# tal-amir/fsw-gnn

Measured on AMD Instinct MI355X. Metric: edges*slices/sec FSW_conv forward, 1M-node/10M-edge, 256 slices, higher is better.
Workload: dtype f32; 1 GPU; BASELINE config 3: ER multigraph 1000000 nodes / 10000000 edges (9999936 after coalesce), 128 feat, 256 slices, FSW_conv(128->128, embed_dim=257), full forward incl. CSR build and Linear layer; nodes=1000000, edges=10000000, edges_coalesced=9999936, slices=256, features=128, parallelism=single GPU

## Files before the change

### fsw_gnn_amd/_lib.py

```python
import ctypes
import os

_HERE = os.path.dirname(os.path.abspath(__file__))
LIB_PATH = os.environ.get("FSW_HIP_LIBRARY") or os.path.join(_HERE, "libfsw_hip.so")

FSW_ABI_VERSION = 6
REG_MAX_DEG = 32
LDS_MAX_DEG = 2048
MID_SIZES = (40, 48, 64, 80, 96, 128, 160, 192, 256)
NUM_LDS_BINS = 3
NUM_HUB_BINS = 4
HUB_MAX_DEG = 32768
CART_SPLIT_LINES = 1
CART_SPLIT_BWD_LINES = 2
CART_SPLIT_W_LINES = 4
CART_W_MAX_LINE = 16384
BIN_MID0 = REG_MAX_DEG + 1
NUM_BINS = REG_MAX_DEG + 1 + len(MID_SIZES) + NUM_LDS_BINS + NUM_HUB_BINS + 1
NUM_STATS = 8
STAT_FLAGS, STAT_MAX_DEGREE, STAT_NUM_ZERO, STAT_NUM_REG, STAT_NUM_LDS, STAT_NUM_GLOBAL, STAT_NNZ, STAT_USER = 0, 1, 2, 3, 4, 5, 6, 7
BIN_BLOCK_ROWS, MAX_ROW_CHUNKS = 2048, 256
FLAG_INDEX_RANGE, FLAG_W_NONFINITE, FLAG_W_NEGATIVE, FLAG_X_NONFINITE = 1, 2, 4, 8

c_i64, c_i32, c_f32, c_vp, c_sz = ctypes.c_int64, ctypes.c_int32, ctypes.c_float, ctypes.c_void_p, ctypes.c_size_t
# ... 32 lines not shown
        ("unit_table", c_vp), ("ldt", c_i64), ("out", c_vp), ("ldo", c_i64), ("bias", c_vp), ("out_scale", ctypes.c_double),
        ("mass_fn", c_i32), ("flags", c_i32), ("mass_scale", ctypes.c_double), ("g", c_vp), ("ldg", c_i64),
        ("gkey", c_vp), ("ldk", c_i64), ("gfreq", c_vp), ("gw", c_vp), ("scratch", c_vp), ("scratch_bytes", c_sz),
    ]


_SIGNATURES = {
    "fsw_abi_version": (ctypes.c_int, []),
    "fsw_arch": (ctypes.c_char_p, []),
    "fsw_last_error": (ctypes.c_char_p, []),
    "fsw_graph_workspace_bytes": (c_sz, [c_i64, c_i64]),
    "fsw_graph_build_coalesced": (ctypes.c_int, [c_vp, c_vp, c_vp, c_vp, ctypes.c_int, c_i64, c_i64, c_i64, c_vp, c_vp, c_vp, c_vp, c_vp,
                                                 c_vp, c_vp, c_vp, c_vp, c_vp, c_sz, c_vp]),
    "fsw_graph_build": (ctypes.c_int, [c_vp, c_vp, c_vp, c_i64, c_i64, c_i64, c_i64, c_vp, c_vp, c_vp, c_vp, c_vp, c_vp, c_vp, c_vp, c_sz, c_vp]),
    "fsw_graph_build_two_level": (ctypes.c_int, [c_vp, c_vp, c_vp, c_i64, c_i64, c_i64, c_i64, c_vp, c_vp, c_vp, c_vp, c_vp, c_vp, c_vp, c_vp, c_sz, c_vp]),
    "fsw_project_f32": (ctypes.c_int, [c_vp, c_i64, ctypes.c_int, c_i64, c_vp, ctypes.c_int, c_i64, c_vp, c_i64, c_vp, c_i64, c_vp, c_vp]),
    "fsw_gemm_tn_workspace_bytes": (c_sz, [ctypes.c_int, ctypes.c_int]),
    "fsw_gemm_tn_f32": (ctypes.c_int, [c_vp, c_i64, c_vp, c_i64, c_i64, ctypes.c_int, ctypes.c_int, c_vp, c_i64, c_f32, c_vp, c_sz, c_vp]),
    "fsw_unit_table_rows": (c_sz, [ctypes.c_int]),
    "fsw_unit_coeff_table": (ctypes.c_int, [c_vp, ctypes.c_int, ctypes.c_int, c_vp, c_i64, c_vp]),
    "fsw_embed_scratch_bytes": (c_sz, [c_i64]),
    "fsw_embed_f32": (ctypes.c_int, [ctypes.POINTER(EmbedArgs), c_vp]),
    "fsw_conv_fused_lds_bytes": (c_sz, [ctypes.c_int, ctypes.c_int]),
    "fsw_packed_linear_floats": (c_sz, [ctypes.c_int, ctypes.c_int]),
    "fsw_pack_linear_f32": (ctypes.c_int, [c_vp, c_i64, ctypes.c_int, ctypes.c_int, ctypes.c_int, c_vp, c_vp, ctypes.c_int, c_vp, c_i64, c_vp]),
    "fsw_project_linear_f32": (ctypes.c_int, [c_vp, c_i64, ctypes.c_int, c_i64, c_vp, ctypes.c_int, c_i64, c_vp, c_i64,
                                              c_vp, ctypes.c_int, c_i64, c_vp, c_vp, c_i64, c_vp, c_vp, c_vp]),
    "fsw_conv_fused_f32": (ctypes.c_int, [ctypes.POINTER(EmbedArgs), c_vp, c_i64, c_vp, ctypes.c_int, c_vp, c_i64, ctypes.c_int,
                                          ctypes.c_int, c_f32, c_vp, c_i64, c_vp]),
    "fsw_add_bias_act_f32": (ctypes.c_int, [c_vp, c_i64, c_vp, c_i64, c_vp, c_i64, ctypes.c_int, ctypes.c_int, c_f32, c_vp]),
# ... 75 lines not shown
```

### fsw_gnn_amd/csrc/graph_build.hip

```cpp
#include <algorithm>
#include <atomic>
#include "fsw_common.h"
#include "graph_ws.h"

namespace fsw {

#ifndef FSW_RS_THREADS
#define FSW_RS_THREADS 512
#endif
constexpr int kRsThreads = FSW_RS_THREADS;
constexpr int kRsItems = kRsTile / kRsThreads;
static_assert(kRsThreads * kRsItems == kRsTile, "a tile is a whole number of rounds");
constexpr int kRsWaves = kRsThreads / kWave;

__device__ __forceinline__ int wave_inclusive_scan(int v) {
#pragma unroll
  for (int off = 1; off < kWave; off <<= 1) {
    int t = __shfl_up(v, off);
    if (lane_id() >= off) v += t;
  }
  return v;
}

__device__ __forceinline__ int block_exclusive_scan(int v, int* total) {
// ... 38 lines not shown
  }
}

__global__ void __launch_bounds__(kScanThreads) k_scan_apply(int32_t* __restrict__ data, int64_t n,
                                                             const int32_t* __restrict__ block_sums) {
  int64_t base = (int64_t)blockIdx.x * kScanTile + (int64_t)threadIdx.x * kScanItems;
  int v[kScanItems];
  int s = 0;
#pragma unroll
  for (int i = 0; i < kScanItems; ++i) {
    v[i] = base + i < n ? data[base + i] : 0;
    s += v[i];
  }
  int tot;
  int ex = block_exclusive_scan(s, &tot) + block_sums[blockIdx.x];
#pragma unroll
  for (int i = 0; i < kScanItems; ++i) {
    if (base + i < n) data[base + i] = ex;
    ex += v[i];
  }
}

static int exclusive_scan_i32(int32_t* data, int64_t n, int32_t* block_sums, int64_t block_sums_cap, hipStream_t stream) {
  const int64_t nb = ceil_div(n, kScanTile);
  FSW_REQUIRE(nb <= block_sums_cap, "exclusive_scan_i32: %lld elements need %lld block sums, the workspace holds %lld",
              (long long)n, (long long)nb, (long long)block_sums_cap);
  k_scan_partial<<<(unsigned)nb, kScanThreads, 0, stream>>>(data, n, block_sums);
  FSW_LAUNCH_CHECK();
  k_scan_block_sums<<<1, kScanThreads, 0, stream>>>(block_sums, nb);
  FSW_LAUNCH_CHECK();
// ... 184 lines not shown
      sval[lpos] = val[i];
    }
  }
  __syncthreads();
  const int64_t tile0 = (int64_t)blockIdx.x * kRsTile;
  const int count = (int)min((int64_t)kRsTile, num_edges - tile0);
  for (int i = threadIdx.x; i < count; i += kRsThreads) {
    const uint32_t k = skey[i];
    const uint32_t d = (k >> shift) & mask;
    const int64_t pos = (int64_t)gbase[d] + (i - dstart[d]);
    keys_out[pos] = k;
    vals_out[pos] = sval[i];
  }
}

template <class VAL>
__global__ void __launch_bounds__(256) k_finish_csr(const uint32_t* __restrict__ keys, const VAL* __restrict__ vals,
                                                    int64_t num_edges, int64_t num_rows, int32_t* __restrict__ rowptr,
                                                    int32_t* __restrict__ col, float* __restrict__ w) {
  for (int64_t i = (int64_t)blockIdx.x * blockDim.x + threadIdx.x; i <= num_edges; i += (int64_t)gridDim.x * blockDim.x) {
    const int64_t prev = i == 0 ? -1 : (int64_t)keys[i - 1];
    const int64_t cur = i == num_edges ? num_rows : (int64_t)keys[i];
    for (int64_t r = prev + 1; r <= cur && r <= num_rows; ++r) rowptr[r] = (int32_t)i;
    if (i < num_edges && cur < num_rows) {
      const VAL v = vals[i];
      col[i] = (int32_t)(uint32_t)v;
      if constexpr (sizeof(VAL) == 8) w[i] = __uint_as_float((uint32_t)(v >> 32));
    }
  }
}
// ... 71 lines not shown
      bin_cursor[c * FSW_NUM_BINS + b] = acc;
      if (b >= 1 && b <= FSW_REG_MAX_DEG) reg += cnt[b];
      if (b >= FSW_BIN_MID0 && b < FSW_BIN_HUB0) mid += cnt[b];
      acc += cnt[b];
    }
    bs[FSW_NUM_BINS] = acc;
    if (cnt[0]) atomicAdd(&stats[FSW_STAT_NUM_ZERO_DEG], cnt[0]);
    if (reg) atomicAdd(&stats[FSW_STAT_NUM_REG], reg);
    if (mid) atomicAdd(&stats[FSW_STAT_NUM_LDS], mid);
    int glob = 0;
    for (int b = FSW_BIN_HUB0; b <= FSW_BIN_GLOBAL; ++b) glob += cnt[b];
    if (glob) atomicAdd(&stats[FSW_STAT_NUM_GLOBAL], glob);
  }
}

__global__ void __launch_bounds__(256) k_bin_rows(const int32_t* __restrict__ rowptr, int64_t n, int64_t chunk_rows,
                                                  int32_t* __restrict__ bin_cursor, int32_t* __restrict__ perm,
                                                  int32_t* __restrict__ invperm) {
  __shared__ int lcount[FSW_NUM_BINS];
  __shared__ int lbase[FSW_NUM_BINS];
  if (threadIdx.x < FSW_NUM_BINS) lcount[threadIdx.x] = 0;
  __syncthreads();
  const int64_t r0 = (int64_t)blockIdx.x * kBinRowsPerBlock + threadIdx.x;
  int bin[kBinItems], rank[kBinItems];
#pragma unroll
  for (int i = 0; i < kBinItems; ++i) {
    const int64_t r = r0 + (int64_t)i * 256;
    const bool valid = r < n;
    bin[i] = valid ? degree_bin(rowptr[r + 1] - rowptr[r]) : 0;
    const unsigned long long peers = match_bin(bin[i], valid);
// ... 4 lines not shown
  }
  __syncthreads();
  const int64_t chunk = ((int64_t)blockIdx.x * kBinRowsPerBlock) / chunk_rows;
  if (threadIdx.x < FSW_NUM_BINS && lcount[threadIdx.x])
    lbase[threadIdx.x] = atomicAdd(&bin_cursor[chunk * FSW_NUM_BINS + threadIdx.x], lcount[threadIdx.x]);
  __syncthreads();
#pragma unroll
  for (int i = 0; i < kBinItems; ++i) {
    const int64_t r = r0 + (int64_t)i * 256;
    if (r < n) {
      const int pos = lbase[bin[i]] + rank[i];
      perm[pos] = (int32_t)r;
      if (invperm) invperm[r] = pos;
    }
  }
}

static int key_bits(int64_t range_a) {
  int keybits = 1;
  while ((1ll << keybits) <= range_a) ++keybits;
  return keybits;
}

template <class VAL, bool EID>
static int radix_sort_pairs(const int64_t* first_a, const int64_t* first_b, const float* edge_w, bool from_keys,
                            int64_t num_edges, int64_t range_a, int64_t range_b, int32_t* stats, GraphWs& g, int* cur_io,
                            hipStream_t stream, int lo_bit = 0, int max_bits = 8, int* last_bits = nullptr) {
  const int keybits = key_bits(range_a) - lo_bit;
  const int npass = (keybits + max_bits - 1) / max_bits;
  const int bits = (keybits + npass - 1) / npass;
  if (last_bits) *last_bits = bits;
  const int64_t ntiles = ceil_div(num_edges, kRsTile);
  int cur = *cur_io;
  for (int pass = 0; pass < npass; ++pass) {
    const int shift = lo_bit + pass * bits;
    const int ndigits = 1 << bits;
// ... 79 lines not shown
    col[p] = (int32_t)senders[eid[i]];
    w[p] = (float)wsum;
  }
}

__global__ void __launch_bounds__(256) k_rowptr_from_keys(const uint32_t* __restrict__ keyc, const int32_t* __restrict__ nnz_ptr,
                                                          int64_t num_rows, int32_t* __restrict__ rowptr) {
  const int64_t nnz = *nnz_ptr;
  for (int64_t i = (int64_t)blockIdx.x * blockDim.x + threadIdx.x; i <= nnz; i += (int64_t)gridDim.x * blockDim.x) {
    const int64_t prev = i == 0 ? -1 : (int64_t)keyc[i - 1];
    const int64_t cur = i == nnz ? num_rows : (int64_t)keyc[i];
    for (int64_t r = prev + 1; r <= cur && r <= num_rows; ++r) rowptr[r] = (int32_t)i;
  }
}

static int finish_bins(int32_t* rowptr, int64_t num_rows, int64_t chunk_rows, int32_t* perm, int32_t* invperm, int32_t* bin_start,
                       int32_t* stats, GraphWs& g, hipStream_t stream) {
  if (chunk_rows <= 0) chunk_rows = ceil_div(num_rows, kBinRowsPerBlock) * kBinRowsPerBlock;
  const int num_chunks = (int)ceil_div(num_rows, chunk_rows);
  const int row_blocks = (int)ceil_div(num_rows, kBinRowsPerBlock);
  k_bin_count<<<row_blocks, 256, 0, stream>>>(rowptr, num_rows, chunk_rows, g.bin_count, stats);
  FSW_LAUNCH_CHECK();
  k_bin_offsets<<<1, kMaxRowChunks, 0, stream>>>(g.bin_count, bin_start, g.bin_cursor, stats, num_chunks, rowptr, num_rows);
  FSW_LAUNCH_CHECK();
  k_bin_rows<<<row_blocks, 256, 0, stream>>>(rowptr, num_rows, chunk_rows, g.bin_cursor, perm, invperm);
  FSW_LAUNCH_CHECK();
  return 0;
}

constexpr int kBucketWaves = 8;
#ifndef FSW_BUCKET_ROW_BITS
#define FSW_BUCKET_ROW_BITS 11
#endif
constexpr int kBucketMaxRowBits = FSW_BUCKET_ROW_BITS;
constexpr int kBucketAhead = 8;

template <class VAL>
__global__ void __launch_bounds__(kBucketWaves * kWave) k_bucket_rows(const uint32_t* __restrict__ keys, const VAL* __restrict__ vals,
                                                                      const int32_t* __restrict__ bstart, int64_t bstride, int ntable,
                                                                      int64_t num_edges, int64_t num_rows, int rb,
                                                                      int32_t* __restrict__ rowptr, int32_t* __restrict__ col,
                                                                      float* __restrict__ w, int stage_cap) {
  extern __shared__ int bsm[];
  const int R = 1 << rb;
  const uint32_t rmask = (uint32_t)R - 1u;
  int* wcnt = bsm;
  int* tot = bsm + kBucketWaves * R;
  VAL* stage = reinterpret_cast<VAL*>(bsm + (kBucketWaves + 1) * R);
  __shared__ int wsum[kBucketWaves];
// ... 110 lines not shown
      }
    }
  }
  if (staged) {
    __syncthreads();
    const int64_t sent = num_rows - (int64_t)b * R;
    const int nvalid = (sent >= 0 && sent < R) ? tot[sent] : (int)(e - s);
    for (int i = threadIdx.x; i < nvalid; i += blockDim.x) {
      const VAL v = stage[i];
      col[s + i] = (int32_t)(uint32_t)v;
      if constexpr (sizeof(VAL) == 8) w[s + i] = __uint_as_float((uint32_t)(v >> 32));
    }
  }
}

__global__ void __launch_bounds__(256) k_bucket_starts(const uint32_t* __restrict__ keys, int64_t num_edges, int rb, int64_t nbuckets,
                                                       int32_t* __restrict__ bstart) {
  for (int64_t i = (int64_t)blockIdx.x * blockDim.x + threadIdx.x; i <= num_edges; i += (int64_t)gridDim.x * blockDim.x) {
    const int64_t prev = i == 0 ? -1 : (int64_t)(keys[i - 1] >> rb);
    const int64_t cur = i == num_edges ? nbuckets : (int64_t)(keys[i] >> rb);
    for (int64_t q = prev + 1; q <= cur && q <= nbuckets; ++q) bstart[q] = (int32_t)i;
  }
}

static bool two_level_ok(int64_t num_rows, int64_t num_edges) {
  if (num_rows < (1 << 15) || num_edges < (1 << 18)) return false;
  const int64_t nbuckets = ceil_div(num_rows + 1, (int64_t)1 << kBucketMaxRowBits);
  return num_edges / nbuckets <= (1 << 16);
}

template <class VAL>
static int sort_and_finish_two_level(const int64_t* recipients, const int64_t* senders, const float* edge_w, int64_t num_edges,
                                     int64_t num_rows, int64_t num_cols, int32_t* rowptr, int32_t* col, float* w, int32_t* stats,
                                     GraphWs& g, hipStream_t stream) {
  const int rb = std::min(kBucketMaxRowBits, key_bits(num_rows));
  const int64_t nbuckets = ceil_div(num_rows + 1, (int64_t)1 << rb);
  const int64_t ntiles = ceil_div(num_edges, kRsTile);
  int cur = 0, bits = 0;
  const int upper = key_bits(num_rows) - rb;
  int rc = radix_sort_pairs<VAL, false>(recipients, senders, edge_w, false, num_edges, num_rows, num_cols, stats, g, &cur, stream, rb, 9, &bits);
  if (rc) return rc;
  const int32_t* bstart = g.counts;
  int64_t bstride = ntiles;
  int ntable = 1 << bits;
  if (bits != upper) {
    const int blocks = (int)std::min<int64_t>(ceil_div(num_edges + 1, 256), 256 * 32);
    k_bucket_starts<<<blocks, 256, 0, stream>>>(g.keys[cur], num_edges, rb, nbuckets, g.block_sums_big);
    FSW_LAUNCH_CHECK();
    bstart = g.block_sums_big;
    bstride = 1;
    ntable = (int)nbuckets + 1;
  }
  const size_t tables = sizeof(int) * (size_t)(kBucketWaves + 1) * ((size_t)1 << rb);
  const size_t room = (size_t)160 * 1024 - 1024 - tables;
  const int64_t avg = ceil_div(num_edges, nbuckets);
  const int64_t want = avg + avg / 32 + 256;
  const int stage_cap = (want * (int64_t)sizeof(VAL) <= (int64_t)room) ? (int)(room / sizeof(VAL)) : 0;
  const size_t lds = tables + (size_t)stage_cap * sizeof(VAL);
  FSW_SET_MAX_LDS_ONCE((&k_bucket_rows<VAL>), 160 * 1024 - 1024);
  k_bucket_rows<VAL><<<(unsigned)nbuckets, kBucketWaves * kWave, lds, stream>>>(g.keys[cur], reinterpret_cast<const VAL*>(g.vals[cur]), bstart,
                                                                              bstride, ntable, num_edges, num_rows, rb, rowptr, col, w,
                                                                              stage_cap);
  FSW_LAUNCH_CHECK();
  return 0;
}

__global__ void __launch_bounds__(256) k_entry_keys(const int32_t* __restrict__ col, int64_t nnz, int64_t num_cols,
                                                    uint32_t* __restrict__ keys, uint32_t* __restrict__ vals) {
  for (int64_t i = (int64_t)blockIdx.x * blockDim.x + threadIdx.x; i < nnz; i += (int64_t)gridDim.x * blockDim.x) {
    const int32_t c = col[i];
    keys[i] = (c < 0 || c >= num_cols) ? (uint32_t)num_cols : (uint32_t)c;
    vals[i] = (uint32_t)i;
  }
}

static int check_chunks(int64_t num_rows, int64_t chunk_rows) {
  FSW_REQUIRE(chunk_rows >= 0 && chunk_rows % kBinRowsPerBlock == 0,
// ... 19 lines not shown
  hipStream_t stream = reinterpret_cast<hipStream_t>(stream_);
  FSW_REQUIRE(num_rows >= 1 && num_rows < (1ll << 31) - 1 && num_cols >= 1 && num_cols < (1ll << 31) && num_edges >= 0 &&
                  num_edges < (1ll << 31) - kRsTile,
              "fsw_graph_build: sizes must satisfy 1 <= rows, cols < 2^31 and 0 <= edges < 2^31 (got %lld, %lld, %lld)",
              (long long)num_rows, (long long)num_cols, (long long)num_edges);
  FSW_REQUIRE(workspace && workspace_bytes >= fsw_graph_workspace_bytes(num_rows, num_edges),
              "fsw_graph_build: workspace too small");
  FSW_REQUIRE(rowptr && perm && bin_start && stats && (num_edges == 0 || (col && recipients && senders)),
              "fsw_graph_build: null pointer");
  FSW_REQUIRE(!edge_w || w, "fsw_graph_build: edge_w given but w is null");
  if (int rc = check_chunks(num_rows, chunk_rows)) return rc;
  GraphWs g = carve(workspace, num_edges, num_rows);

  FSW_CHECK_HIP(hipMemsetAsync(g.bin_count, 0, kBinTableBytes, stream));
  FSW_CHECK_HIP(hipMemsetAsync(stats, 0, sizeof(int32_t) * FSW_NUM_STATS, stream));
  if (num_edges == 0) {
    FSW_CHECK_HIP(hipMemsetAsync(rowptr, 0, sizeof(int32_t) * (size_t)(num_rows + 1), stream));
  } else if (two_level && two_level_ok(num_rows, num_edges)) {
    int rc = edge_w ? sort_and_finish_two_level<unsigned long long>(recipients, senders, edge_w, num_edges, num_rows, num_cols, rowptr, col, w, stats, g, stream)
                    : sort_and_finish_two_level<uint32_t>(recipients, senders, edge_w, num_edges, num_rows, num_cols, rowptr, col, w, stats, g, stream);
    if (rc) return rc;
  } else {
    int rc = edge_w ? sort_and_finish<unsigned long long>(recipients, senders, edge_w, num_edges, num_rows, num_cols, rowptr, col, w, stats, g, stream)
                    : sort_and_finish<uint32_t>(recipients, senders, edge_w, num_edges, num_rows, num_cols, rowptr, col, w, stats, g, stream);
    if (rc) return rc;
  }
  return finish_bins(rowptr, num_rows, chunk_rows, perm, invperm, bin_start, stats, g, stream);
}

extern "C" int fsw_graph_build(const int64_t* recipients, const int64_t* senders, const float* edge_w, int64_t num_edges,
                               int64_t num_rows, int64_t num_cols, int64_t chunk_rows, int32_t* rowptr, int32_t* col, float* w,
                               int32_t* perm, int32_t* invperm, int32_t* bin_start, int32_t* stats, void* workspace,
                               size_t workspace_bytes, fsw_stream_t stream) {
  return graph_build_impl(recipients, senders, edge_w, num_edges, num_rows, num_cols, chunk_rows, rowptr, col, w, perm, invperm, bin_start,
                          stats, workspace, workspace_bytes, stream, false);
}

extern "C" int fsw_graph_build_two_level(const int64_t* recipients, const int64_t* senders, const float* edge_w, int64_t num_edges,
                                         int64_t num_rows, int64_t num_cols, int64_t chunk_rows, int32_t* rowptr, int32_t* col, float* w,
                                         int32_t* perm, int32_t* invperm, int32_t* bin_start, int32_t* stats, void* workspace,
                                         size_t workspace_bytes, fsw_stream_t stream) {
  return graph_build_impl(recipients, senders, edge_w, num_edges, num_rows, num_cols, chunk_rows, rowptr, col, w, perm, invperm, bin_start,
// ... 78 lines not shown
```

### fsw_gnn_amd/csrc/graph_ws.h

```cpp
#pragma once
#include <stddef.h>
#include <stdint.h>
#include "../../include/fsw_hip.h"

namespace fsw {

constexpr int kScanThreads = 256;
constexpr int kScanItems = 16;
constexpr int kScanTile = kScanThreads * kScanItems;
constexpr int kRsTile = 4096;
constexpr int kRsMaxDigits = 512;
constexpr int kMaxRowChunks = 256;
constexpr size_t kBinTableBytes = sizeof(int32_t) * kMaxRowChunks * FSW_NUM_BINS;
constexpr size_t kWsAlign = 256;
static_assert(kMaxRowChunks == FSW_MAX_ROW_CHUNKS, "include/fsw_hip.h documents the number of row chunks");

inline size_t ws_align_up(size_t v, size_t a) { return (v + a - 1) / a * a; }
inline size_t ws_ceil_div(size_t a, size_t b) { return (a + b - 1) / b; }

enum GraphWsRegion {
  kWsKeys0, kWsKeys1, kWsVals0, kWsVals1, kWsCounts, kWsBlockSums, kWsBlockSumsBig, kWsBinCount, kWsBinCursor, kWsNumRegions
};

struct GraphWsLayout {
// ... 46 lines not shown
  GraphWs g;
  g.keys[0] = reinterpret_cast<uint32_t*>(at(kWsKeys0));
  g.keys[1] = reinterpret_cast<uint32_t*>(at(kWsKeys1));
  g.vals[0] = at(kWsVals0);
  g.vals[1] = at(kWsVals1);
  g.counts = reinterpret_cast<int32_t*>(at(kWsCounts));
  g.block_sums = reinterpret_cast<int32_t*>(at(kWsBlockSums));
  g.block_sums_cap = l.block_sums_cap;
  g.block_sums_big = reinterpret_cast<int32_t*>(at(kWsBlockSumsBig));
  g.bin_count = reinterpret_cast<int32_t*>(at(kWsBinCount));
  g.bin_cursor = reinterpret_cast<int32_t*>(at(kWsBinCursor));
  g.total = l.total;
  return g;
}

}
```

### include/fsw_hip.h

```cpp
#ifndef FSW_HIP_H
#define FSW_HIP_H

#include <stdbool.h>
#include <stddef.h>
#include <stdint.h>

#ifdef __cplusplus
extern "C" {
#endif

typedef void* fsw_stream_t;

#define FSW_ABI_VERSION 6

#define FSW_REG_MAX_DEG 32
#define FSW_NUM_MID_BINS 9
#define FSW_MID_SIZES {40, 48, 64, 80, 96, 128, 160, 192, 256}
#define FSW_MID_MAX_DEG 256
#define FSW_MID_MAX_DEG_WEIGHTED 128
#define FSW_LDS_MAX_DEG 2048
#define FSW_HUB_MAX_DEG 32768
#define FSW_CART_W_MAX_LINE 16384
#define FSW_BIN_MID0 (FSW_REG_MAX_DEG + 1)
#define FSW_NUM_LDS_BINS 3
// ... 21 lines not shown
int fsw_abi_version(void);
const char* fsw_arch(void);
const char* fsw_last_error(void);

#define FSW_BIN_BLOCK_ROWS 2048
#define FSW_MAX_ROW_CHUNKS 256
size_t fsw_graph_workspace_bytes(int64_t num_rows, int64_t num_edges);
int fsw_graph_build(const int64_t* recipients, const int64_t* senders, const float* edge_w,
                    int64_t num_edges, int64_t num_rows, int64_t num_cols, int64_t chunk_rows,
                    int32_t* rowptr, int32_t* col, float* w, int32_t* perm, int32_t* invperm, int32_t* bin_start,
                    int32_t* stats, void* workspace, size_t workspace_bytes, fsw_stream_t stream);
int fsw_graph_build_two_level(const int64_t* recipients, const int64_t* senders, const float* edge_w,
                    int64_t num_edges, int64_t num_rows, int64_t num_cols, int64_t chunk_rows,
                    int32_t* rowptr, int32_t* col, float* w, int32_t* perm, int32_t* invperm, int32_t* bin_start,
                    int32_t* stats, void* workspace, size_t workspace_bytes, fsw_stream_t stream);

int fsw_graph_build_coalesced(const int64_t* recipients, const int64_t* senders, const float* edge_w,
                              const float* edge_feat, int d_edge, int64_t num_edges, int64_t num_rows, int64_t num_cols,
                              int32_t* rowptr, int32_t* col, float* w, float* ef, int32_t* slot_of_edge, int32_t* perm,
                              int32_t* invperm, int32_t* bin_start, int32_t* stats, void* workspace, size_t workspace_bytes,
                              fsw_stream_t stream);

int fsw_project_f32(const float* X, int64_t n, int d, int64_t ldx, const float* V, int S, int64_t ldv,
                    float* Xp, int64_t ldp, float* x_copy, int64_t ld_copy, int32_t* stats, fsw_stream_t stream);

size_t fsw_gemm_tn_workspace_bytes(int M, int N);
int fsw_gemm_tn_f32(const float* A, int64_t lda, const float* B, int64_t ldb, int64_t K, int M, int N, float* C, int64_t ldc, float beta,
                    void* workspace, size_t workspace_bytes, fsw_stream_t stream);

size_t fsw_unit_table_rows(int max_deg);
// ... 185 lines not shown
```

Measured before the change: 884.4 billion edges*slices/sec.

## Pack row and sender into one word for single-pass two-level CSR build

For unweighted graphs where one partition pass covers the upper row bits and row-low bits plus sender bits fit in 32 bits, the two-level CSR build now packs each edge into a single 32-bit word. It uses a new upsweep/downsweep over larger tiles with vectorized index loads, then a packed bucket-rows kernel that also accumulates the bin counts, so the separate bin-count pass is skipped and a one-wave-per-chunk offsets kernel is used instead. This is meant to cut memory traffic and kernel launches in graph construction. In exchange it adds a second code path with tighter eligibility conditions and a plan helper exposed through the API.

```diff
diff --git a/fsw_gnn_amd/_lib.py b/fsw_gnn_amd/_lib.py
--- a/fsw_gnn_amd/_lib.py
+++ b/fsw_gnn_amd/_lib.py
@@ -70,6 +70,7 @@
                                                  c_vp, c_vp, c_vp, c_vp, c_vp, c_sz, c_vp]),
     "fsw_graph_build": (ctypes.c_int, [c_vp, c_vp, c_vp, c_i64, c_i64, c_i64, c_i64, c_vp, c_vp, c_vp, c_vp, c_vp, c_vp, c_vp, c_vp, c_sz, c_vp]),
     "fsw_graph_build_two_level": (ctypes.c_int, [c_vp, c_vp, c_vp, c_i64, c_i64, c_i64, c_i64, c_vp, c_vp, c_vp, c_vp, c_vp, c_vp, c_vp, c_vp, c_sz, c_vp]),
+    "fsw_graph_build_plan": (ctypes.c_int, [c_i64, c_i64, c_i64, ctypes.c_int, ctypes.POINTER(c_i32)]),
     "fsw_project_f32": (ctypes.c_int, [c_vp, c_i64, ctypes.c_int, c_i64, c_vp, ctypes.c_int, c_i64, c_vp, c_i64, c_vp, c_i64, c_vp, c_vp]),
     "fsw_gemm_tn_workspace_bytes": (c_sz, [ctypes.c_int, ctypes.c_int]),
     "fsw_gemm_tn_f32": (ctypes.c_int, [c_vp, c_i64, c_vp, c_i64, c_i64, ctypes.c_int, ctypes.c_int, c_vp, c_i64, c_f32, c_vp, c_sz, c_vp]),
diff --git a/fsw_gnn_amd/csrc/graph_build.hip b/fsw_gnn_amd/csrc/graph_build.hip
--- a/fsw_gnn_amd/csrc/graph_build.hip
+++ b/fsw_gnn_amd/csrc/graph_build.hip
@@ -2,6 +2,7 @@
 #include <atomic>
 #include "fsw_common.h"
 #include "graph_ws.h"
+#include "graph_plan.h"
 
 namespace fsw {
 
@@ -76,6 +77,24 @@
   }
   int tot;
   int ex = block_exclusive_scan(s, &tot) + block_sums[blockIdx.x];
+#pragma unroll
+  for (int i = 0; i < kScanItems; ++i) {
+    if (base + i < n) data[base + i] = ex;
+    ex += v[i];
+  }
+}
+
+__global__ void __launch_bounds__(kScanThreads) k_scan_one(int32_t* __restrict__ data, int64_t n) {
+  const int64_t base = (int64_t)threadIdx.x * kScanItems;
+  int v[kScanItems];
+  int s = 0;
+#pragma unroll
+  for (int i = 0; i < kScanItems; ++i) {
+    v[i] = base + i < n ? data[base + i] : 0;
+    s += v[i];
+  }
+  int tot;
+  int ex = block_exclusive_scan(s, &tot);
 #pragma unroll
   for (int i = 0; i < kScanItems; ++i) {
     if (base + i < n) data[base + i] = ex;
@@ -290,6 +309,182 @@
   }
 }
 
+constexpr int kPackItems = kPackTile / kRsThreads;
+constexpr int kPackAhead = 8;
+static_assert(kRsThreads * kPackItems == kPackTile && kPackItems % kPackAhead == 0, "a packed tile is a whole number of load groups");
+static_assert(kRsMaxDigits <= (1 << 16), "the digit of an edge is kept in 16 bits");
+constexpr size_t kPackLdsBytes = sizeof(int) * (size_t)(kRsWaves + 2) * kRsMaxDigits + (sizeof(uint32_t) + sizeof(uint16_t)) * (size_t)kPackTile;
+
+__device__ __forceinline__ uint32_t key_of(int64_t r, int64_t c, int64_t num_rows, int64_t num_cols, int& flags) {
+  if (r < 0 || r >= num_rows || c < 0 || c >= num_cols) {
+    flags |= FSW_FLAG_INDEX_RANGE;
+    return (uint32_t)num_rows;
+  }
+  return (uint32_t)r;
+}
+
+template <bool VEC>
+__global__ void __launch_bounds__(kRsThreads) k_pack_upsweep(const int64_t* __restrict__ recipients, const int64_t* __restrict__ senders,
+                                                             int64_t num_edges, int64_t num_rows, int64_t num_cols, int shift, int ndigits,
+                                                             int32_t* __restrict__ counts , int64_t ntiles,
+                                                             int32_t* __restrict__ stats) {
+  __shared__ int hist[kRsMaxDigits];
+  for (int d = threadIdx.x; d < ndigits; d += kRsThreads) hist[d] = 0;
+  __syncthreads();
+  const int64_t tile0 = (int64_t)blockIdx.x * kPackTile;
+  const uint32_t mask = (uint32_t)ndigits - 1;
+  int flags = 0;
+  if constexpr (VEC) {
+    constexpr int kPairs = kPackItems / 2, kPairsAhead = kPackAhead / 2;
+    static_assert(kPackItems % 2 == 0 && kPairs % kPairsAhead == 0, "pairs of edges in whole load groups");
+#pragma unroll
+    for (int h = 0; h < kPairs / kPairsAhead; ++h) {
+      uint32_t key[kPairsAhead][2];
+#pragma unroll
+      for (int i = 0; i < kPairsAhead; ++i) {
+        const int64_t e = tile0 + 2 * ((int64_t)(h * kPairsAhead + i) * kRsThreads + threadIdx.x);
+        key[i][0] = key[i][1] = 0xffffffffu;
+        if (e + 1 < num_edges) {
+          const longlong2 r = *reinterpret_cast<const longlong2*>(recipients + e);
+          const longlong2 c = *reinterpret_cast<const longlong2*>(senders + e);
+          key[i][0] = key_of(r.x, c.x, num_rows, num_cols, flags);
+          key[i][1] = key_of(r.y, c.y, num_rows, num_cols, flags);
+        } else if (e < num_edges) {
+          key[i][0] = key_of(recipients[e], senders[e], num_rows, num_cols, flags);
+        }
+      }
+#pragma unroll
+      for (int i = 0; i < kPairsAhead; ++i) {
+        const int64_t e = tile0 + 2 * ((int64_t)(h * kPairsAhead + i) * kRsThreads + threadIdx.x);
+        if (e < num_edges) atomicAdd(&hist[(key[i][0] >> shift) & mask], 1);
+        if (e + 1 < num_edges) atomicAdd(&hist[(key[i][1] >> shift) & mask], 1);
+      }
+    }
+  } else {
+#pragma unroll
+    for (int h = 0; h < kPackItems / kPackAhead; ++h) {
+      uint32_t key[kPackAhead];
+#pragma unroll
+      for (int i = 0; i < kPackAhead; ++i) {
+        const int64_t e = tile0 + (int64_t)(h * kPackAhead + i) * kRsThreads + threadIdx.x;
+        key[i] = 0xffffffffu;
+        if (e < num_edges) key[i] = key_of(recipients[e], senders[e], num_rows, num_cols, flags);
+      }
+#pragma unroll
+      for (int i = 0; i < kPackAhead; ++i)
+        if (tile0 + (int64_t)(h * kPackAhead + i) * kRsThreads + threadIdx.x < num_edges) atomicAdd(&hist[(key[i] >> shift) & mask], 1);
+    }
+  }
+  __syncthreads();
+  for (int d = threadIdx.x; d < ndigits; d += kRsThreads) counts[(int64_t)d * ntiles + blockIdx.x] = hist[d];
+  if (flags) atomicOr(&stats[FSW_STAT_FLAGS], flags);
+}
+
+__global__ void __launch_bounds__(kRsThreads) k_pack_downsweep(const int64_t* __restrict__ recipients, const int64_t* __restrict__ senders,
+                                                               int64_t num_edges, int64_t num_rows, int64_t num_cols, int rb, int cb,
+                                                               int nbits, const int32_t* __restrict__ bases ,
+                                                               int64_t ntiles, uint32_t* __restrict__ words_out) {
+  extern __shared__ int psm[];
+  int* wcnt = psm;
+  int* dstart = psm + kRsWaves * kRsMaxDigits;
+  int* gbase = dstart + kRsMaxDigits;
+  uint32_t* sword = reinterpret_cast<uint32_t*>(gbase + kRsMaxDigits);
+  uint16_t* sdig = reinterpret_cast<uint16_t*>(sword + kPackTile);
+  const int ndigits = 1 << nbits;
+  const uint32_t mask = (uint32_t)ndigits - 1, rmask = (1u << rb) - 1u;
+  const int lane = lane_id(), wv = threadIdx.x >> 6;
+  int* mine = wcnt + wv * kRsMaxDigits;
+  for (int d = threadIdx.x; d < ndigits; d += kRsThreads) {
+#pragma unroll
+    for (int w = 0; w < kRsWaves; ++w) wcnt[w * kRsMaxDigits + d] = 0;
+    gbase[d] = bases[(int64_t)d * ntiles + blockIdx.x];
+  }
+  __syncthreads();
+
+  const int64_t wave0 = (int64_t)blockIdx.x * kPackTile + (int64_t)wv * (kPackItems * kWave);
+  uint32_t word[kPackItems];
+  int dig[kPackItems], rank[kPackItems];
+  int dummy = 0;
+#pragma unroll
+  for (int h = 0; h < kPackItems / kPackAhead; ++h) {
+    uint32_t key[kPackAhead], snd[kPackAhead];
+#pragma unroll
+    for (int u = 0; u < kPackAhead; ++u) {
+      const int64_t e = wave0 + (int64_t)(h * kPackAhead + u) * kWave + lane;
+      key[u] = 0xffffffffu;
+      snd[u] = 0u;
+      if (e < num_edges) {
+        key[u] = load_key<true>(recipients, senders, nullptr, e, num_rows, num_cols, dummy);
+        snd[u] = (uint32_t)senders[e];
+      }
+    }
+#pragma unroll
+    for (int u = 0; u < kPackAhead; ++u) {
+      const int i = h * kPackAhead + u;
+      const bool ok = wave0 + (int64_t)i * kWave + lane < num_edges;
+      const uint32_t d = (key[u] >> rb) & mask;
+      word[i] = pack_edge(key[u], rmask, cb, (int64_t)key[u] < num_rows ? snd[u] : 0u);
+      dig[i] = (int)d;
+      const unsigned long long peers = match_digit<9>(d, ok);
+      const int leader = __ffsll((long long)peers) - 1;
+      const int below = __popcll(peers & ((1ull << lane) - 1ull));
+      int prev = 0;
+      if (ok && lane == leader) {
+        prev = mine[d];
+        mine[d] = prev + __popcll(peers);
+      }
+      prev = __shfl(prev, leader);
+      rank[i] = prev + below;
+    }
+  }
+  __syncthreads();
+  for (int d = threadIdx.x; d < ndigits; d += kRsThreads) {
+    int acc = 0;
+#pragma unroll
+    for (int w = 0; w < kRsWaves; ++w) {
+      const int c = wcnt[w * kRsMaxDigits + d];
+      wcnt[w * kRsMaxDigits + d] = acc;
+      acc += c;
+    }
+    dstart[d] = acc;
+  }
+  __syncthreads();
+  if (threadIdx.x < kWave) {
+    constexpr int kPer = kRsMaxDigits / kWave;
+    int v[kPer], s = 0;
+#pragma unroll
+    for (int j = 0; j < kPer; ++j) {
+      const int d = lane * kPer + j;
+      v[j] = d < ndigits ? dstart[d] : 0;
+      s += v[j];
+    }
+    int ex = wave_inclusive_scan(s) - s;
+#pragma unroll
+    for (int j = 0; j < kPer; ++j) {
+      const int d = lane * kPer + j;
+      if (d < ndigits) dstart[d] = ex;
+      ex += v[j];
+    }
+  }
+  __syncthreads();
+#pragma unroll
+  for (int i = 0; i < kPackItems; ++i) {
+    const int64_t e = wave0 + (int64_t)i * kWave + lane;
+    if (e < num_edges) {
+      const int lpos = dstart[dig[i]] + mine[dig[i]] + rank[i];
+      sword[lpos] = word[i];
+      sdig[lpos] = (uint16_t)dig[i];
+    }
+  }
+  __syncthreads();
+  const int64_t tile0 = (int64_t)blockIdx.x * kPackTile;
+  const int count = (int)min((int64_t)kPackTile, num_edges - tile0);
+  for (int i = threadIdx.x; i < count; i += kRsThreads) {
+    const int d = sdig[i];
+    words_out[(int64_t)gbase[d] + (i - dstart[d])] = sword[i];
+  }
+}
+
 template <class VAL>
 __global__ void __launch_bounds__(256) k_finish_csr(const uint32_t* __restrict__ keys, const VAL* __restrict__ vals,
                                                     int64_t num_edges, int64_t num_rows, int32_t* __restrict__ rowptr,
@@ -391,6 +586,40 @@
   }
 }
 
+static_assert(FSW_NUM_BINS <= kWave, "one lane per bin");
+__global__ void __launch_bounds__(kWave) k_bin_offsets_wave(const int32_t* __restrict__ bin_count, int32_t* __restrict__ bin_start,
+                                                            int32_t* __restrict__ bin_cursor, int32_t* __restrict__ stats,
+                                                            const int32_t* __restrict__ rowptr, int64_t num_rows) {
+  const int c = blockIdx.x, b = threadIdx.x;
+  if (c == 0 && b == 0) stats[FSW_STAT_NNZ] = rowptr[num_rows];
+  int before = 0;
+  for (int i = b; i < c * FSW_NUM_BINS; i += kWave) before += bin_count[i];
+#pragma unroll
+  for (int off = 32; off > 0; off >>= 1) before += __shfl_xor(before, off);
+  const int cnt = b < FSW_NUM_BINS ? bin_count[c * FSW_NUM_BINS + b] : 0;
+  const int inc = wave_inclusive_scan(cnt);
+  if (b < FSW_NUM_BINS) {
+    bin_start[c * (FSW_NUM_BINS + 1) + b] = before + inc - cnt;
+    bin_cursor[c * FSW_NUM_BINS + b] = before + inc - cnt;
+  }
+  if (b == FSW_NUM_BINS - 1) bin_start[c * (FSW_NUM_BINS + 1) + FSW_NUM_BINS] = before + inc;
+  int reg = (b >= 1 && b <= FSW_REG_MAX_DEG) ? cnt : 0;
+  int mid = (b >= FSW_BIN_MID0 && b < FSW_BIN_HUB0) ? cnt : 0;
+  int glob = (b >= FSW_BIN_HUB0 && b <= FSW_BIN_GLOBAL) ? cnt : 0;
+#pragma unroll
+  for (int off = 32; off > 0; off >>= 1) {
+    reg += __shfl_xor(reg, off);
+    mid += __shfl_xor(mid, off);
+    glob += __shfl_xor(glob, off);
+  }
+  if (b == 0) {
+    if (cnt) atomicAdd(&stats[FSW_STAT_NUM_ZERO_DEG], cnt);
+    if (reg) atomicAdd(&stats[FSW_STAT_NUM_REG], reg);
+    if (mid) atomicAdd(&stats[FSW_STAT_NUM_LDS], mid);
+    if (glob) atomicAdd(&stats[FSW_STAT_NUM_GLOBAL], glob);
+  }
+}
+
 __global__ void __launch_bounds__(256) k_bin_rows(const int32_t* __restrict__ rowptr, int64_t n, int64_t chunk_rows,
                                                   int32_t* __restrict__ bin_cursor, int32_t* __restrict__ perm,
                                                   int32_t* __restrict__ invperm) {
@@ -425,12 +654,6 @@
       if (invperm) invperm[r] = pos;
     }
   }
-}
-
-static int key_bits(int64_t range_a) {
-  int keybits = 1;
-  while ((1ll << keybits) <= range_a) ++keybits;
-  return keybits;
 }
 
 template <class VAL, bool EID>
@@ -540,25 +763,29 @@
   }
 }
 
+static int64_t one_chunk_if_zero(int64_t num_rows, int64_t chunk_rows) {
+  return chunk_rows > 0 ? chunk_rows : ceil_div(num_rows, kBinRowsPerBlock) * kBinRowsPerBlock;
+}
+
 static int finish_bins(int32_t* rowptr, int64_t num_rows, int64_t chunk_rows, int32_t* perm, int32_t* invperm, int32_t* bin_start,
-                       int32_t* stats, GraphWs& g, hipStream_t stream) {
-  if (chunk_rows <= 0) chunk_rows = ceil_div(num_rows, kBinRowsPerBlock) * kBinRowsPerBlock;
+                       int32_t* stats, GraphWs& g, hipStream_t stream, bool counted = false) {
+  chunk_rows = one_chunk_if_zero(num_rows, chunk_rows);
   const int num_chunks = (int)ceil_div(num_rows, chunk_rows);
   const int row_blocks = (int)ceil_div(num_rows, kBinRowsPerBlock);
-  k_bin_count<<<row_blocks, 256, 0, stream>>>(rowptr, num_rows, chunk_rows, g.bin_count, stats);
-  FSW_LAUNCH_CHECK();
-  k_bin_offsets<<<1, kMaxRowChunks, 0, stream>>>(g.bin_count, bin_start, g.bin_cursor, stats, num_chunks, rowptr, num_rows);
+  if (!counted) {
+    k_bin_count<<<row_blocks, 256, 0, stream>>>(rowptr, num_rows, chunk_rows, g.bin_count, stats);
+    FSW_LAUNCH_CHECK();
+  }
+  if (counted)
+    k_bin_offsets_wave<<<num_chunks, kWave, 0, stream>>>(g.bin_count, bin_start, g.bin_cursor, stats, rowptr, num_rows);
+  else
+    k_bin_offsets<<<1, kMaxRowChunks, 0, stream>>>(g.bin_count, bin_start, g.bin_cursor, stats, num_chunks, rowptr, num_rows);
   FSW_LAUNCH_CHECK();
   k_bin_rows<<<row_blocks, 256, 0, stream>>>(rowptr, num_rows, chunk_rows, g.bin_cursor, perm, invperm);
   FSW_LAUNCH_CHECK();
   return 0;
 }
 
-constexpr int kBucketWaves = 8;
-#ifndef FSW_BUCKET_ROW_BITS
-#define FSW_BUCKET_ROW_BITS 11
-#endif
-constexpr int kBucketMaxRowBits = FSW_BUCKET_ROW_BITS;
 constexpr int kBucketAhead = 8;
 
 template <class VAL>
@@ -699,6 +926,147 @@
   }
 }
 
+static_assert((1 << kBucketMaxRowBits) == FSW_BIN_BLOCK_ROWS, "a bucket of the two-level build is one bin block: it never straddles a row chunk");
+
+__global__ void __launch_bounds__(kBucketWaves * kWave) k_bucket_rows_packed(const uint32_t* __restrict__ words, const int32_t* __restrict__ bstart,
+                                                                             int64_t bstride, int ntable, int64_t num_edges, int64_t num_rows,
+                                                                             int rb, int cb, int32_t* __restrict__ rowptr,
+                                                                             int32_t* __restrict__ col, int stage_cap, int64_t chunk_rows,
+                                                                             int32_t* __restrict__ bin_count, int32_t* __restrict__ stats) {
+  extern __shared__ int bsm[];
+  const int R = 1 << rb;
+  int* wcnt = bsm;
+  int* tot = bsm + kBucketWaves * R;
+  uint32_t* stage = reinterpret_cast<uint32_t*>(bsm + (kBucketWaves + 1) * R);
+  __shared__ int wsum[kBucketWaves];
+  __shared__ int lbin[FSW_NUM_BINS];
+  __shared__ int lmax;
+  const int b = blockIdx.x, lane = lane_id(), wv = threadIdx.x >> 6;
+  const int64_t s = bstart[(int64_t)b * bstride];
+  const int64_t e = b + 1 < ntable ? (int64_t)bstart[(int64_t)(b + 1) * bstride] : num_edges;
+  for (int i = threadIdx.x; i < kBucketWaves * R; i += blockDim.x) wcnt[i] = 0;
+  if (threadIdx.x < FSW_NUM_BINS) lbin[threadIdx.x] = 0;
+  if (threadIdx.x == 0) lmax = 0;
+  __syncthreads();
+  const int64_t L = ceil_div(e - s, (int64_t)kBucketWaves * kWave) * kWave;
+  const int64_t w0 = min(s + wv * L, e), w1 = min(w0 + L, e);
+  int* mine = wcnt + wv * R;
+  const bool staged = e - s <= stage_cap;
+  {
+    uint32_t kn[kBucketAhead];
+#pragma unroll
+    for (int u = 0; u < kBucketAhead; ++u) kn[u] = w0 + lane + u * kWave < w1 ? words[w0 + lane + u * kWave] : 0u;
+    for (int64_t i = w0 + lane; i < w1; i += kBucketAhead * kWave) {
+      uint32_t kk[kBucketAhead];
+#pragma unroll
+      for (int u = 0; u < kBucketAhead; ++u) kk[u] = kn[u];
+      const int64_t nx = i + kBucketAhead * kWave;
+      if (nx - lane < w1) {
+#pragma unroll
+        for (int u = 0; u < kBucketAhead; ++u) kn[u] = nx + u * kWave < w1 ? words[nx + u * kWave] : 0u;
+      }
+#pragma unroll
+      for (int u = 0; u < kBucketAhead; ++u)
+        if (i + u * kWave < w1) atomicAdd(&mine[edge_row(kk[u], cb)], 1);
+    }
+  }
+  __syncthreads();
+  for (int r = threadIdx.x; r < R; r += blockDim.x) {
+    int acc = 0;
+#pragma unroll
+    for (int q = 0; q < kBucketWaves; ++q) {
+      const int c = wcnt[q * R + r];
+      wcnt[q * R + r] = acc;
+      acc += c;
+    }
+    tot[r] = acc;
+  }
+  __syncthreads();
+  {
+    constexpr int kPerMax = (1 << kBucketMaxRowBits) / (kBucketWaves * kWave);
+    const int per = max(R / (int)blockDim.x, 1);
+    const int r0 = threadIdx.x * per;
+    int v[kPerMax], sum = 0, mx = 0;
+#pragma unroll
+    for (int j = 0; j < kPerMax; ++j) {
+      v[j] = (j < per && r0 + j < R) ? tot[r0 + j] : 0;
+      sum += v[j];
+      const bool valid = j < per && r0 + j < R && (int64_t)b * R + r0 + j < num_rows;
+      const int bin = degree_bin(valid ? v[j] : 0);
+      if (valid) mx = max(mx, v[j]);
+      const unsigned long long peers = match_bin(bin, valid);
+      if (valid && lane == __ffsll((long long)peers) - 1) atomicAdd(&lbin[bin], __popcll(peers));
+    }
+#pragma unroll
+    for (int off = 32; off > 0; off >>= 1) mx = max(mx, __shfl_xor(mx, off));
+    if (lane == 0 && mx) atomicMax(&lmax, mx);
+    const int inc = wave_inclusive_scan(sum);
+    if (lane == kWave - 1) wsum[wv] = inc;
+    __syncthreads();
+    int base = 0;
+#pragma unroll
+    for (int q = 0; q < kBucketWaves; ++q)
+      if (q < wv) base += wsum[q];
+    int ex = base + inc - sum;
+#pragma unroll
+    for (int j = 0; j < kPerMax; ++j)
+      if (j < per && r0 + j < R) {
+        tot[r0 + j] = ex;
+        const int64_t row = (int64_t)b * R + r0 + j;
+        if (row <= num_rows) rowptr[row] = (int32_t)(s + ex);
+        ex += v[j];
+      }
+    const int64_t chunk = ((int64_t)b * R) / chunk_rows;
+    if (threadIdx.x < FSW_NUM_BINS && lbin[threadIdx.x]) atomicAdd(&bin_count[chunk * FSW_NUM_BINS + threadIdx.x], lbin[threadIdx.x]);
+    if (threadIdx.x == 0 && lmax) atomicMax(&stats[FSW_STAT_MAX_DEGREE], lmax);
+  }
+  __syncthreads();
+  uint32_t wordn[kBucketAhead];
+  auto load_group = [&](int64_t g) {
+#pragma unroll
+    for (int u = 0; u < kBucketAhead; ++u) {
+      const int64_t i = g + u * kWave + lane;
+      wordn[u] = i < w1 ? words[i] : 0u;
+    }
+  };
+  load_group(w0);
+  const int64_t rows_here = num_rows - (int64_t)b * R;
+  for (int64_t g0 = w0; g0 < w1; g0 += kBucketAhead * kWave) {
+    uint32_t wordv[kBucketAhead];
+#pragma unroll
+    for (int u = 0; u < kBucketAhead; ++u) wordv[u] = wordn[u];
+    if (g0 + kBucketAhead * kWave < w1) load_group(g0 + kBucketAhead * kWave);
+#pragma unroll
+    for (int u = 0; u < kBucketAhead; ++u) {
+      if (g0 + u * kWave >= w1) break;
+      const bool ok = g0 + u * kWave + lane < w1;
+      const uint32_t k = edge_row(wordv[u], cb);
+      const unsigned long long peers = match_digit<kBucketMaxRowBits>(k, ok);
+      const int leader = __ffsll((long long)peers) - 1;
+      const int below = __popcll(peers & ((1ull << lane) - 1ull));
+      int prev = 0;
+      if (ok && lane == leader) {
+        prev = mine[k];
+        mine[k] = prev + __popcll(peers);
+      }
+      prev = __shfl(prev, leader);
+      if (ok && (int64_t)k < rows_here) {
+        const int lpos = tot[k] + prev + below;
+        const uint32_t sender = edge_sender(wordv[u], cb);
+        if (staged)
+          stage[lpos] = sender;
+        else
+          col[s + lpos] = (int32_t)sender;
+      }
+    }
+  }
+  if (staged) {
+    __syncthreads();
+    const int nvalid = (rows_here >= 0 && rows_here < R) ? tot[rows_here] : (int)(e - s);
+    for (int i = threadIdx.x; i < nvalid; i += blockDim.x) col[s + i] = (int32_t)stage[i];
+  }
+}
+
 __global__ void __launch_bounds__(256) k_bucket_starts(const uint32_t* __restrict__ keys, int64_t num_edges, int rb, int64_t nbuckets,
                                                        int32_t* __restrict__ bstart) {
   for (int64_t i = (int64_t)blockIdx.x * blockDim.x + threadIdx.x; i <= num_edges; i += (int64_t)gridDim.x * blockDim.x) {
@@ -708,27 +1076,22 @@
   }
 }
 
-static bool two_level_ok(int64_t num_rows, int64_t num_edges) {
-  if (num_rows < (1 << 15) || num_edges < (1 << 18)) return false;
-  const int64_t nbuckets = ceil_div(num_rows + 1, (int64_t)1 << kBucketMaxRowBits);
-  return num_edges / nbuckets <= (1 << 16);
-}
-
+static_assert(kPartitionBits == 9, "graph_ws.h: the literal handed to radix_sort_pairs below");
 template <class VAL>
 static int sort_and_finish_two_level(const int64_t* recipients, const int64_t* senders, const float* edge_w, int64_t num_edges,
                                      int64_t num_rows, int64_t num_cols, int32_t* rowptr, int32_t* col, float* w, int32_t* stats,
-                                     GraphWs& g, hipStream_t stream) {
-  const int rb = std::min(kBucketMaxRowBits, key_bits(num_rows));
-  const int64_t nbuckets = ceil_div(num_rows + 1, (int64_t)1 << rb);
+                                     GraphWs& g, hipStream_t stream, const TwoLevelPlan& p) {
+  const int rb = p.rb;
+  const int64_t nbuckets = p.nbuckets;
   const int64_t ntiles = ceil_div(num_edges, kRsTile);
   int cur = 0, bits = 0;
-  const int upper = key_bits(num_rows) - rb;
   int rc = radix_sort_pairs<VAL, false>(recipients, senders, edge_w, false, num_edges, num_rows, num_cols, stats, g, &cur, stream, rb, 9, &bits);
   if (rc) return rc;
+  FSW_REQUIRE(bits == p.bits, "fsw_graph_build_two_level: the partition ran passes of %d bits, the plan says %d", bits, p.bits);
   const int32_t* bstart = g.counts;
   int64_t bstride = ntiles;
   int ntable = 1 << bits;
-  if (bits != upper) {
+  if (bits != p.upper) {
     const int blocks = (int)std::min<int64_t>(ceil_div(num_edges + 1, 256), 256 * 32);
     k_bucket_starts<<<blocks, 256, 0, stream>>>(g.keys[cur], num_edges, rb, nbuckets, g.block_sums_big);
     FSW_LAUNCH_CHECK();
@@ -736,16 +1099,42 @@
     bstride = 1;
     ntable = (int)nbuckets + 1;
   }
-  const size_t tables = sizeof(int) * (size_t)(kBucketWaves + 1) * ((size_t)1 << rb);
-  const size_t room = (size_t)160 * 1024 - 1024 - tables;
-  const int64_t avg = ceil_div(num_edges, nbuckets);
-  const int64_t want = avg + avg / 32 + 256;
-  const int stage_cap = (want * (int64_t)sizeof(VAL) <= (int64_t)room) ? (int)(room / sizeof(VAL)) : 0;
-  const size_t lds = tables + (size_t)stage_cap * sizeof(VAL);
   FSW_SET_MAX_LDS_ONCE((&k_bucket_rows<VAL>), 160 * 1024 - 1024);
-  k_bucket_rows<VAL><<<(unsigned)nbuckets, kBucketWaves * kWave, lds, stream>>>(g.keys[cur], reinterpret_cast<const VAL*>(g.vals[cur]), bstart,
-                                                                              bstride, ntable, num_edges, num_rows, rb, rowptr, col, w,
-                                                                              stage_cap);
+  k_bucket_rows<VAL><<<(unsigned)nbuckets, kBucketWaves * kWave, p.lds, stream>>>(g.keys[cur], reinterpret_cast<const VAL*>(g.vals[cur]), bstart,
+                                                                                bstride, ntable, num_edges, num_rows, rb, rowptr, col, w,
+                                                                                p.stage_cap);
+  FSW_LAUNCH_CHECK();
+  return 0;
+}
+
+static int sort_and_finish_packed(const int64_t* recipients, const int64_t* senders, int64_t num_edges, int64_t num_rows, int64_t num_cols,
+                                  int64_t chunk_rows, int32_t* rowptr, int32_t* col, int32_t* stats, GraphWs& g, hipStream_t stream,
+                                  const TwoLevelPlan& p) {
+  const int ndigits = 1 << p.bits;
+  FSW_REQUIRE(p.packed && ndigits <= kRsMaxDigits && (int64_t)ndigits * p.ntiles <= (int64_t)kRsMaxDigits * ceil_div(num_edges, kRsTile),
+              "fsw_graph_build_two_level: the packed count table does not fit the workspace");
+  uint32_t* words = g.keys[1];
+  if (((reinterpret_cast<uintptr_t>(recipients) | reinterpret_cast<uintptr_t>(senders)) & 15) == 0)
+    k_pack_upsweep<true><<<(unsigned)p.ntiles, kRsThreads, 0, stream>>>(recipients, senders, num_edges, num_rows, num_cols, p.rb, ndigits,
+                                                                       g.counts, p.ntiles, stats);
+  else
+    k_pack_upsweep<false><<<(unsigned)p.ntiles, kRsThreads, 0, stream>>>(recipients, senders, num_edges, num_rows, num_cols, p.rb, ndigits,
+                                                                        g.counts, p.ntiles, stats);
+  FSW_LAUNCH_CHECK();
+  if ((int64_t)ndigits * p.ntiles <= kScanTile) {
+    k_scan_one<<<1, kScanThreads, 0, stream>>>(g.counts, (int64_t)ndigits * p.ntiles);
+    FSW_LAUNCH_CHECK();
+  } else if (int rc = exclusive_scan_i32(g.counts, (int64_t)ndigits * p.ntiles, g.block_sums, g.block_sums_cap, stream)) {
+    return rc;
+  }
+  FSW_SET_MAX_LDS_ONCE((&k_pack_downsweep), kPackLdsBytes);
+  k_pack_downsweep<<<(unsigned)p.ntiles, kRsThreads, kPackLdsBytes, stream>>>(recipients, senders, num_edges, num_rows, num_cols, p.rb, p.cb,
+                                                                             p.bits, g.counts, p.ntiles, words);
+  FSW_LAUNCH_CHECK();
+  FSW_SET_MAX_LDS_ONCE((&k_bucket_rows_packed), 160 * 1024 - 1024);
+  k_bucket_rows_packed<<<(unsigned)p.nbuckets, kBucketWaves * kWave, p.lds, stream>>>(words, g.counts, p.ntiles, ndigits, num_edges, num_rows,
+                                                                                     p.rb, p.cb, rowptr, col, p.stage_cap,
+                                                                                     one_chunk_if_zero(num_rows, chunk_rows), g.bin_count, stats);
   FSW_LAUNCH_CHECK();
   return 0;
 }
@@ -795,18 +1184,30 @@
 
   FSW_CHECK_HIP(hipMemsetAsync(g.bin_count, 0, kBinTableBytes, stream));
   FSW_CHECK_HIP(hipMemsetAsync(stats, 0, sizeof(int32_t) * FSW_NUM_STATS, stream));
+  const bool try_two = two_level && num_edges > 0 && two_level_ok(num_rows, num_edges);
+  const TwoLevelPlan p = try_two ? two_level_plan(num_rows, num_cols, num_edges, edge_w != nullptr) : TwoLevelPlan{};
+  const bool counted = try_two && p.packed;
   if (num_edges == 0) {
     FSW_CHECK_HIP(hipMemsetAsync(rowptr, 0, sizeof(int32_t) * (size_t)(num_rows + 1), stream));
-  } else if (two_level && two_level_ok(num_rows, num_edges)) {
-    int rc = edge_w ? sort_and_finish_two_level<unsigned long long>(recipients, senders, edge_w, num_edges, num_rows, num_cols, rowptr, col, w, stats, g, stream)
-                    : sort_and_finish_two_level<uint32_t>(recipients, senders, edge_w, num_edges, num_rows, num_cols, rowptr, col, w, stats, g, stream);
+  } else if (try_two) {
+    int rc = p.packed ? sort_and_finish_packed(recipients, senders, num_edges, num_rows, num_cols, chunk_rows, rowptr, col, stats, g, stream, p)
+             : edge_w ? sort_and_finish_two_level<unsigned long long>(recipients, senders, edge_w, num_edges, num_rows, num_cols, rowptr, col, w, stats, g, stream, p)
+                      : sort_and_finish_two_level<uint32_t>(recipients, senders, edge_w, num_edges, num_rows, num_cols, rowptr, col, w, stats, g, stream, p);
     if (rc) return rc;
   } else {
     int rc = edge_w ? sort_and_finish<unsigned long long>(recipients, senders, edge_w, num_edges, num_rows, num_cols, rowptr, col, w, stats, g, stream)
                     : sort_and_finish<uint32_t>(recipients, senders, edge_w, num_edges, num_rows, num_cols, rowptr, col, w, stats, g, stream);
     if (rc) return rc;
   }
-  return finish_bins(rowptr, num_rows, chunk_rows, perm, invperm, bin_start, stats, g, stream);
+  return finish_bins(rowptr, num_rows, chunk_rows, perm, invperm, bin_start, stats, g, stream, counted);
+}
+
+extern "C" int fsw_graph_build_plan(int64_t num_rows, int64_t num_cols, int64_t num_edges, int weighted, int32_t* out) {
+  FSW_REQUIRE(out && num_rows >= 1 && num_rows < (1ll << 31) - 1 && num_cols >= 1 && num_cols < (1ll << 31) && num_edges >= 0 &&
+                  num_edges < (1ll << 31) - kRsTile,
+              "fsw_graph_build_plan: null pointer or sizes outside 1 <= rows, cols < 2^31, 0 <= edges < 2^31");
+  graph_plan_words(num_rows, num_cols, num_edges, weighted != 0, out);
+  return 0;
 }
 
 extern "C" int fsw_graph_build(const int64_t* recipients, const int64_t* senders, const float* edge_w, int64_t num_edges,
diff --git a/fsw_gnn_amd/csrc/graph_plan.h b/fsw_gnn_amd/csrc/graph_plan.h
--- /dev/null
+++ b/fsw_gnn_amd/csrc/graph_plan.h
@@ -0,0 +1,97 @@
+#pragma once
+#include <stdint.h>
+#include "graph_ws.h"
+
+#if defined(__HIPCC__)
+#define FSW_PLAN_HD __host__ __device__ inline
+#else
+#define FSW_PLAN_HD inline
+#endif
+
+namespace fsw {
+
+constexpr int kPackTile = 8192;
+static_assert(kPackTile % kRsTile == 0, "the packed count table ([digits][tiles of kPackTile]) fits the region sized for kRsTile");
+
+inline int key_bits(int64_t range) {
+  int keybits = 1;
+  while ((1ll << keybits) <= range) ++keybits;
+  return keybits;
+}
+
+FSW_PLAN_HD uint32_t pack_edge(uint32_t row, uint32_t rmask, int cb, uint32_t sender) { return ((row & rmask) << cb) | sender; }
+FSW_PLAN_HD uint32_t edge_row(uint32_t word, int cb) { return word >> cb; }
+FSW_PLAN_HD uint32_t edge_sender(uint32_t word, int cb) { return word & ((1u << cb) - 1u); }
+
+inline int sender_bits(int64_t num_cols) { return key_bits(num_cols > 1 ? num_cols - 1 : 0); }
+
+inline bool packed_ok(bool weighted, int pass_bits, int upper_bits, int rb, int cb) {
+  return !weighted && pass_bits == upper_bits && rb + cb <= 32;
+}
+
+enum GraphPlanWord {
+  kPlanTwoLevel,
+  kPlanPacked,
+  kPlanTile,
+  kPlanStageCap,
+  kPlanPasses,
+  kPlanRowBits,
+  kPlanSenderBits,
+  kPlanBuckets,
+  kPlanNumWords
+};
+
+static_assert(kPlanNumWords == FSW_GRAPH_PLAN_WORDS, "include/fsw_hip.h documents the words of the plan");
+
+struct TwoLevelPlan {
+  int rb, upper, passes, bits, cb;
+  bool packed;
+  int tile;
+  int64_t ntiles, nbuckets;
+  int stage_cap;
+  size_t tables, lds;
+};
+
+inline TwoLevelPlan two_level_plan(int64_t num_rows, int64_t num_cols, int64_t num_edges, bool weighted) {
+  TwoLevelPlan p;
+  const int kb = key_bits(num_rows);
+  p.rb = kBucketMaxRowBits < kb ? kBucketMaxRowBits : kb;
+  p.nbuckets = (num_rows + 1 + ((int64_t)1 << p.rb) - 1) >> p.rb;
+  p.upper = kb - p.rb;
+  p.passes = (p.upper + kPartitionBits - 1) / kPartitionBits;
+  p.bits = p.passes ? (p.upper + p.passes - 1) / p.passes : 0;
+  p.cb = sender_bits(num_cols);
+  p.packed = p.passes == 1 && packed_ok(weighted, p.bits, p.upper, p.rb, p.cb);
+  p.tile = p.packed ? kPackTile : kRsTile;
+  p.ntiles = (int64_t)ws_ceil_div((size_t)num_edges, (size_t)p.tile);
+  const size_t vsize = weighted ? sizeof(unsigned long long) : sizeof(uint32_t);
+  const size_t tables = sizeof(int) * (size_t)(kBucketWaves + 1) * ((size_t)1 << p.rb);
+  const size_t room = bucket_stage_room(tables);
+  const int64_t avg = (num_edges + p.nbuckets - 1) / p.nbuckets;
+  const int64_t want = avg + avg / 32 + 256;
+  p.stage_cap = (want * (int64_t)vsize <= (int64_t)room) ? (int)(room / vsize) : 0;
+  p.tables = tables;
+  p.lds = tables + (size_t)p.stage_cap * vsize;
+  return p;
+}
+
+inline void graph_plan_words(int64_t num_rows, int64_t num_cols, int64_t num_edges, bool weighted, int32_t* out) {
+  for (int i = 0; i < kPlanNumWords; ++i) out[i] = 0;
+  if (num_edges == 0 || !two_level_ok(num_rows, num_edges)) return;
+  const TwoLevelPlan p = two_level_plan(num_rows, num_cols, num_edges, weighted);
+  out[kPlanTwoLevel] = 1;
+  out[kPlanPacked] = p.packed;
+  out[kPlanTile] = p.tile;
+  out[kPlanStageCap] = p.stage_cap;
+  out[kPlanPasses] = p.passes;
+  out[kPlanRowBits] = p.rb;
+  out[kPlanSenderBits] = p.cb;
+  out[kPlanBuckets] = (int32_t)p.nbuckets;
+}
+
+inline bool plan_fits_workspace(const TwoLevelPlan& p, const GraphWsLayout& l) {
+  const size_t n = ((size_t)1 << p.bits) * (size_t)p.ntiles;
+  return sizeof(int32_t) * n <= l.bytes[kWsCounts] && (int64_t)ws_ceil_div(n, kScanTile) <= l.block_sums_cap;
+}
+
+}
diff --git a/fsw_gnn_amd/csrc/graph_ws.h b/fsw_gnn_amd/csrc/graph_ws.h
--- a/fsw_gnn_amd/csrc/graph_ws.h
+++ b/fsw_gnn_amd/csrc/graph_ws.h
@@ -84,4 +84,22 @@
   return g;
 }
 
+constexpr int kBucketWaves = 8;
+#ifndef FSW_BUCKET_ROW_BITS
+#define FSW_BUCKET_ROW_BITS 11
+#endif
+constexpr int kBucketMaxRowBits = FSW_BUCKET_ROW_BITS;
+constexpr int kPartitionBits = 9;
+
+static bool two_level_ok(int64_t num_rows, int64_t num_edges) {
+  if (num_rows < (1 << 15) || num_edges < (1 << 18)) return false;
+  const int64_t nbuckets = (num_rows + 1 + ((int64_t)1 << kBucketMaxRowBits) - 1) >> kBucketMaxRowBits;
+  return num_edges / nbuckets <= (1 << 16);
 }
+
+inline size_t bucket_stage_room(size_t tables) {
+  const size_t room = (size_t)160 * 1024 - 1024 - tables;
+  return room;
+}
+
+}
diff --git a/include/fsw_hip.h b/include/fsw_hip.h
--- a/include/fsw_hip.h
+++ b/include/fsw_hip.h
@@ -59,6 +59,8 @@
                     int64_t num_edges, int64_t num_rows, int64_t num_cols, int64_t chunk_rows,
                     int32_t* rowptr, int32_t* col, float* w, int32_t* perm, int32_t* invperm, int32_t* bin_start,
                     int32_t* stats, void* workspace, size_t workspace_bytes, fsw_stream_t stream);
+#define FSW_GRAPH_PLAN_WORDS 8
+int fsw_graph_build_plan(int64_t num_rows, int64_t num_cols, int64_t num_edges, int weighted, int32_t* out);
 
 int fsw_graph_build_coalesced(const int64_t* recipients, const int64_t* senders, const float* edge_w,
                               const float* edge_feat, int d_edge, int64_t num_edges, int64_t num_rows, int64_t num_cols,
```

New measurement: 909.6 billion edges*slices/sec (median of 6 runs). 2.9% higher.
